# Yxxxb/LAVT-RS

Measured on NVIDIA B200. Metric: LAVT-RS fwd clips/s (8x384^2), higher is better.
Workload: dtype bf16

## Files before the change

### include/lavt_b200.h

```cpp
#ifndef LAVT_B200_H_
#define LAVT_B200_H_

#include <stdint.h>

#ifdef __cplusplus
extern "C" {
#endif

#define LAVT_ABI_VERSION 4

#define LAVT_ERR_SHAPE 1
#define LAVT_ERR_CUDA 2
#define LAVT_ERR_ARCH 3

enum { LAVT_ACT_NONE = 0, LAVT_ACT_GELU = 1, LAVT_ACT_RELU = 2, LAVT_ACT_TANH = 3, LAVT_ACT_SIGMOID = 4 };

typedef struct lavt_win_geom {
  int32_t B, D, H, W;
  int32_t wd, wh, ww;
  int32_t sd, sh, sw;
  int32_t nwd, nwh, nww;
  int32_t N;
  int32_t Wd, Wh, Ww;
} lavt_win_geom_t;

typedef struct lavt_epilogue {
  const float* cscale;
  const float* bias;
  int32_t act;
  int32_t ldm;
  const void* mul;
  const float* resid;
  float* out_f32;
  void* out_bf16;
  int32_t ldo;
  int32_t mul_act;
  const lavt_win_geom_t* win;
  const float* rscale;
  int32_t rscale_rows;
  int32_t pre_mode;
  void* out_pre;
} lavt_epilogue_t;

const char* lavt_last_error(void);
int lavt_abi_version(void);
int lavt_check_device(void);

int lavt_gemm_bf16(const void* A, int64_t lda, const void* Wt, int64_t ldw, int32_t M, int32_t N, int32_t K,
                   const lavt_epilogue_t* epi, void* stream);

int lavt_conv3x3_bf16(const void* x_nhwc, int64_t ldx, int32_t n_img, int32_t H, int32_t W, int32_t Cin,
                      const void* Wt, int32_t Cout, const lavt_epilogue_t* epi, void* stream);

int lavt_conv3d_bf16(const void* x_ndhwc, int64_t ldx, int32_t n_clip, int32_t D, int32_t H, int32_t W, int32_t Cin,
                     const void* Wt, int32_t Cout, const lavt_epilogue_t* epi, void* stream);


int lavt_layernorm_rows(const float* x, int64_t ldx, int64_t M, int32_t C, const float* gamma, const float* beta,
                        float eps, void* out_bf16, float* out_f32, void* stream);

int lavt_layernorm_window_gather(const float* x, int32_t C, const lavt_win_geom_t* geom, const float* gamma,
                                 const float* beta, float eps, void* out_bf16, void* stream);

int lavt_patch_merge_layernorm(const float* x, int32_t B, int32_t D, int32_t H, int32_t W, int32_t C,
                               const float* gamma, const float* beta, float eps, void* out_bf16, void* stream);

int lavt_patch_embed_im2col(const float* x, int64_t stride_b, int64_t stride_c, int64_t stride_t, int32_t B, int32_t T,
                            int32_t H, int32_t W, void* out_bf16, void* stream);

int lavt_window_attention(const void* qkv, const float* table_t, int32_t L, int32_t nH, const lavt_win_geom_t* geom,
                          void* out_bf16, void* stream);
int lavt_window_attention_lse(const void* qkv, const float* table_t, int32_t L, int32_t nH, const lavt_win_geom_t* geom, void* out_bf16,
                              float* lse, void* stream);
int lavt_window_attention_has_lse(const lavt_win_geom_t* geom, int32_t L, int32_t nH);
int lavt_set_attention_impl(int32_t impl);

int64_t lavt_instnorm_workspace_floats(int32_t B, int64_t n, int32_t C);
int lavt_instnorm_stats(const float* x, int32_t B, int64_t n, int32_t C, float eps, float* stats,
                        float* workspace, void* stream);
int lavt_pwam_kv(const float* l, const float* mask, const float* wk, const float* bk, const float* wv, const float* bv,
                 float* k, float* v, int32_t B, int32_t Nl, int32_t Lin, int32_t C, void* stream);
int lavt_lang_project(const float* l, const float* mask, const float* w0, const float* b0, const float* w2, const float* b2, float* stats,
// ... 157 lines not shown
```

### lavt_rs_b200/_cabi.py

```python
from __future__ import annotations

import ctypes as C
import os
from typing import Optional

import torch

_PKG = os.path.dirname(os.path.abspath(__file__))
LIB_PATH = os.environ.get("LAVT_LIB_PATH") or os.path.join(_PKG, "_lib", "liblavt_b200.so")

ACT_NONE, ACT_GELU, ACT_RELU, ACT_TANH, ACT_SIGMOID = 0, 1, 2, 3, 4


class WinGeom(C.Structure):
    _fields_ = [(n, C.c_int32) for n in
                ("B", "D", "H", "W", "wd", "wh", "ww", "sd", "sh", "sw",
                 "nwd", "nwh", "nww", "N", "Wd", "Wh", "Ww")]

    def rows(self) -> int:
        return self.B * self.nwd * self.nwh * self.nww * self.N

    def tokens(self) -> int:
        return self.B * self.D * self.H * self.W

# ... 14 lines not shown
class LavtError(RuntimeError):
    pass


_lib: Optional[C.CDLL] = None


def lib() -> C.CDLL:
    global _lib
    if _lib is not None:
        return _lib
    if not os.path.exists(LIB_PATH):
        raise LavtError(
            f"{LIB_PATH} not found: build it with `python -m lavt_rs_b200.build` "
            "(the B200 path has no CPU / PyTorch fallback)")
    l = C.CDLL(LIB_PATH)
    l.lavt_last_error.restype = C.c_char_p
    _declare(l)
    if l.lavt_abi_version() != ABI_VERSION:
        raise LavtError("liblavt_b200.so ABI version mismatch; rebuild")
    _lib = l
    return l


ABI_VERSION = 4

_i32, _i64, _f32, _vp = C.c_int32, C.c_int64, C.c_float, C.c_void_p
_EP = C.POINTER(Epilogue)
_WG = C.POINTER(WinGeom)

SIGNATURES = {
    "lavt_check_device": [],
    "lavt_gemm_bf16": [_vp, _i64, _vp, _i64, _i32, _i32, _i32, _EP, _vp],
    "lavt_gemm_bf16_smallm": [_vp, _i64, _vp, _i64, _i32, _i32, _i32, _EP, _vp, _i64, _vp],
    "lavt_conv3x3_bf16": [_vp, _i64, _i32, _i32, _i32, _i32, _vp, _i32, _EP, _vp],
    "lavt_conv3d_bf16": [_vp, _i64, _i32, _i32, _i32, _i32, _i32, _vp, _i32, _EP, _vp],
    "lavt_layernorm_rows": [_vp, _i64, _i64, _i32, _vp, _vp, _f32, _vp, _vp, _vp],
    "lavt_layernorm_window_gather": [_vp, _i32, _WG, _vp, _vp, _f32, _vp, _vp],
    "lavt_patch_merge_layernorm": [_vp, _i32, _i32, _i32, _i32, _i32, _vp, _vp, _f32, _vp, _vp],
    "lavt_patch_embed_im2col": [_vp, _i64, _i64, _i64, _i32, _i32, _i32, _i32, _vp, _vp],
    "lavt_window_attention": [_vp, _vp, _i32, _i32, _WG, _vp, _vp],
    "lavt_window_attention_lse": [_vp, _vp, _i32, _i32, _WG, _vp, _vp, _vp],
    "lavt_instnorm_stats": [_vp, _i32, _i64, _i32, _f32, _vp, _vp, _vp],
    "lavt_pwam_kv": [_vp, _vp, _vp, _vp, _vp, _vp, _vp, _vp, _i32, _i32, _i32, _i32, _vp],
    "lavt_lang_project": [_vp, _vp, _vp, _vp, _vp, _vp, _vp, _i32, _i32, _i32, _i32, _vp],
    "lavt_lang_project_bwd": [_vp, _vp, _vp, _vp, _vp, _vp, _vp, _vp, _vp, _vp, _vp, _vp, _i32, _i32, _i32, _i32, _vp],
    "lavt_pwam_attend": [_vp, _vp, _vp, _vp, _vp, _vp, _i32, _i64, _i32, _i32, _i32, _vp],
    "lavt_pwam_mul_norm": [_vp, _vp, _vp, _vp, _i32, _i64, _i32, _vp],
    "lavt_instnorm_sum2": [_vp, _vp, _vp, _vp, _vp, _i32, _i64, _i32, _vp],
    "lavt_bert_embed": [_vp, _vp, _vp, _vp, _vp, _i32, _i32, _i32, _i32, _vp],
    "lavt_bert_attention": [_vp, _vp, _vp, _i32, _i32, _i32, _i32, _vp],
    "lavt_rows_to_channels_first": [_vp, _vp, _i32, _i32, _i32, _vp],
    "lavt_split3_bf16": [_vp, _i64, _vp, _i64, _i32, _vp],
    "lavt_bert_attention_f32": [_vp, _vp, _vp, _i32, _i32, _i32, _i32, _vp],
    "lavt_upsample_concat": [_vp, _i32, _i32, _i32, _vp, _i32, _vp, _i32, _i32, _i32, _vp],
    "lavt_upconv_blend": [_vp, _i32, _i32, _i32, _vp, _vp, _vp, _vp, _i32, _i32, _i32, _vp],
    "lavt_conv1x1_logits": [_vp, _vp, _vp, _vp, _i64, _i32, _vp],
    "lavt_upsample_logits": [_vp, _vp, _i32, _i32, _i32, _i32, _i32, _vp],
    "lavt_nhwc_to_nchw": [_vp, _vp, _i32, _i32, _i32, _vp],
    "lavt_nchw_to_nhwc_bf16": [_vp, _vp, _i32, _i32, _i32, _vp],
    "lavt_gemm_bf16_splitk": [_vp, _i64, _vp, _i64, _i32, _i32, _i32, _i32, _vp, _i64, _vp, _i64, _i32, _vp],
    "lavt_gemm_bf16_wgrad": [_vp, _i64, _vp, _i64, _i64, _i32, _i32, _vp, _i64, _vp, _i64, _i32, _vp],
    "lavt_conv3x3_wgrad": [_vp, _vp, _i32, _i32, _i32, _i32, _i32, _vp, _i64, _vp, _i32, _vp],
    "lavt_conv3d_wgrad": [_vp, _vp, _i32, _i32, _i32, _i32, _i32, _i32, _vp, _i64, _vp, _i32, _vp],
    "lavt_transpose_bf16": [_vp, _i64, _vp, _i64, _i64, _i32, _vp],
    "lavt_colsum_accumulate": [_vp, _i32, _i64, _i64, _i32, _vp, _vp],
# ... 175 lines not shown
        torch.cuda.synchronize()
        out = {}
        for fam, fl, nb, s, e, _tag in self.records:
            d = out.setdefault(fam, {"launches": 0, "ms": 0.0, "flops": 0.0, "bytes": 0.0, "ideal_ms": 0.0})
            d["launches"] += 1
            d["ms"] += s.elapsed_time(e)
            d["flops"] += fl
            d["bytes"] += nb
            if peak_tflops > 0 and peak_gbs > 0:
                d["ideal_ms"] += max(fl / (peak_tflops * 1e12), nb / (peak_gbs * 1e9)) * 1e3
        return out


TIMER = KernelTimer()


def gemm_bf16(a: torch.Tensor, w: torch.Tensor, **epi) -> None:
    _req(a, torch.bfloat16, "a")
    _req(w, torch.bfloat16, "w")
    M, K = a.shape
    N, K2 = w.shape
    if K != K2:
        raise LavtError(f"gemm: K mismatch {K} vs {K2}")
    e = make_epilogue(**epi)
    t0 = TIMER.begin()
    check(lib().lavt_gemm_bf16(a.data_ptr(), a.stride(0), w.data_ptr(), w.stride(0), M, N, K,
                               C.byref(e), stream_ptr()), "lavt_gemm_bf16")
    if t0 is not None:
        nbytes = 2.0 * (M * K + N * K) + M * N * ((4.0 if e.out_f32 else 0.0) + (2.0 if e.out_bf16 else 0.0)
                                                   + (4.0 if e.resid else 0.0) + (2.0 if e.mul else 0.0))
        TIMER.end(t0, "gemm_bf16_tc_kernel", 2.0 * M * N * K, nbytes, f"M{M} N{N} K{K} act{e.act}")


def gemm_bf16_smallm(a: torch.Tensor, w: torch.Tensor, workspace: torch.Tensor, **epi) -> None:
    _req(a, torch.bfloat16, "a")
    _req(w, torch.bfloat16, "w")
    M, K = a.shape
    N, K2 = w.shape
    if K != K2:
        raise LavtError(f"gemm: K mismatch {K} vs {K2}")
    e = make_epilogue(**epi)
    check(lib().lavt_gemm_bf16_smallm(a.data_ptr(), a.stride(0), w.data_ptr(), w.stride(0), M, N, K, C.byref(e),
                                      _c(workspace, torch.float32, "workspace").data_ptr(), workspace.numel(), stream_ptr()),
          "lavt_gemm_bf16_smallm")


def conv3x3_bf16(x_nhwc: torch.Tensor, w_taps: torch.Tensor, **epi) -> None:
    _req(x_nhwc, torch.bfloat16, "x")
    _req(w_taps, torch.bfloat16, "w_taps")
    n_img, H, W, Cin = x_nhwc.shape
    if not x_nhwc.is_contiguous():
        raise LavtError("conv: x must be contiguous NHWC")
    Cout = w_taps.shape[0]
    e = make_epilogue(**epi)
    t0 = TIMER.begin()
    check(lib().lavt_conv3x3_bf16(x_nhwc.data_ptr(), Cin, n_img, H, W, Cin, w_taps.data_ptr(), Cout,
                                  C.byref(e), stream_ptr()), "lavt_conv3x3_bf16")
    npix = n_img * H * W
    TIMER.end(t0, "gemm_bf16_tc_kernel", 2.0 * npix * Cout * 9 * Cin, 2.0 * (npix * Cin + Cout * 9 * Cin + npix * Cout),
              f"conv {n_img}x{H}x{W} Cin{Cin} Cout{Cout}")


def conv3d_bf16(x_ndhwc: torch.Tensor, w_taps: torch.Tensor, **epi) -> None:
    _req(x_ndhwc, torch.bfloat16, "x")
    _req(w_taps, torch.bfloat16, "w_taps")
    n_clip, D, H, W, Cin = x_ndhwc.shape
# ... 778 lines not shown
```

### lavt_rs_b200/csrc/cabi.cu

```cuda
#include "../../include/lavt_b200.h"
#include "common.cuh"
#include "gemm_tc.cuh"
#include "kernels.cuh"

#include <cstring>

namespace lavt {
const char* last_error();
int gemm_dispatch(const void* A, long long lda, const void* Bw, long long ldb, const GemmParams& p,
                  cudaStream_t stream);

static_assert(sizeof(lavt_win_geom_t) == sizeof(WinGeom), "public/private window geometry mismatch");

static int fill_epilogue(GemmParams& p, const lavt_epilogue_t* e) {
  LAVT_REQUIRE(e != nullptr, "epilogue pointer is NULL");
  p.cscale = e->cscale;
  p.bias = e->bias;
  p.act = e->act;
  p.mul = static_cast<const __nv_bfloat16*>(e->mul);
  p.ldm = e->ldm;
  p.mul_act = e->mul_act;
  p.out_pre = static_cast<__nv_bfloat16*>(e->out_pre);
  p.pre_mode = e->pre_mode;
  LAVT_REQUIRE(e->pre_mode == 0 || (e->pre_mode == 1 && e->out_pre && e->act == LAVT_ACT_GELU),
               "epilogue: pre_mode 1 (out_pre = GELU'(pre)) needs out_pre and act = LAVT_ACT_GELU");
  LAVT_REQUIRE(e->mul_act == 0 || (e->mul_act == LAVT_ACT_GELU && e->mul), "epilogue: mul_act must be 0 or LAVT_ACT_GELU with a mul operand");
  p.resid = e->resid;
  p.out_f32 = e->out_f32;
  p.out_bf16 = static_cast<__nv_bfloat16*>(e->out_bf16);
  p.ldo = e->ldo;
  p.rscale = e->rscale;
  p.rs_rows = e->rscale_rows;
  LAVT_REQUIRE(!e->rscale || e->rscale_rows > 0, "epilogue: rscale needs rscale_rows > 0");
  LAVT_REQUIRE(e->act >= 0 && e->act <= 4, "bad activation id %d", e->act);
  if (e->win) {
    p.rowmap = ROWMAP_WINDOW;
    std::memcpy(&p.win, e->win, sizeof(WinGeom));
  } else {
    p.rowmap = ROWMAP_IDENTITY;
  }
  return LAVT_OK;
}
}
// ... 2 lines not shown

extern "C" {

const char* lavt_last_error(void) { return lavt::last_error(); }
int lavt_abi_version(void) { return LAVT_ABI_VERSION; }

int lavt_check_device(void) {
  int dev = 0;
  LAVT_CUDA(cudaGetDevice(&dev));
  cudaDeviceProp prop;
  LAVT_CUDA(cudaGetDeviceProperties(&prop, dev));
  if (prop.major != 10) {
    set_last_error("device %d is sm_%d%d; this library is built for sm_100a only", dev, prop.major, prop.minor);
    return LAVT_ERR_ARCH;
  }
  return LAVT_OK;
}

int lavt_gemm_bf16(const void* A, int64_t lda, const void* Wt, int64_t ldw, int32_t M, int32_t N, int32_t K,
                   const lavt_epilogue_t* epi, void* stream) {
  GemmParams p;
  std::memset(&p, 0, sizeof(p));
  p.M = M; p.N = N; p.K = K;
  int rc = fill_epilogue(p, epi);
  if (rc) return rc;
  if (p.rowmap == ROWMAP_WINDOW) {
    const WinGeom& g = p.win;
    long long rows = 1LL * g.B * g.nwd * g.nwh * g.nww * g.N;
    LAVT_REQUIRE(rows == M, "gemm: window geometry rows %lld != M %d", rows, M);
  }
  return gemm_dispatch(A, lda, Wt, ldw, p, static_cast<cudaStream_t>(stream));
}

static void conv_pick_tile(GemmParams& p, int H, int W) {
  int best_tw = 8; long long best_area = -1;
  for (int tw = 8; tw <= 128; tw *= 2) {
    int th = 128 / tw;
    long long area = 1LL * ((H + th - 1) / th) * th * ((W + tw - 1) / tw) * tw;
    if (best_area < 0 || area < best_area || (area == best_area && tw > best_tw)) { best_area = area; best_tw = tw; }
  }
  p.cTW = best_tw; p.cTH = 128 / best_tw;
  p.cTilesW = (W + p.cTW - 1) / p.cTW;
  p.cTilesH = (H + p.cTH - 1) / p.cTH;
}

int lavt_conv3x3_bf16(const void* x_nhwc, int64_t ldx, int32_t n_img, int32_t H, int32_t W, int32_t Cin,
                      const void* Wt, int32_t Cout, const lavt_epilogue_t* epi, void* stream) {
  GemmParams p;
  std::memset(&p, 0, sizeof(p));
  LAVT_REQUIRE(n_img > 0 && H > 0 && W > 0, "conv: empty input");
  p.M = n_img * H * W; p.N = Cout; p.K = 9 * Cin;
  int rc = fill_epilogue(p, epi);
  if (rc) return rc;
  LAVT_REQUIRE(p.rowmap == ROWMAP_IDENTITY, "conv: window row map not applicable");
  p.rowmap = ROWMAP_CONV;
  p.cH = H; p.cW = W; p.cCin = Cin; p.taps = 9;
  conv_pick_tile(p, H, W);
  return gemm_dispatch(x_nhwc, ldx, Wt, 9LL * Cin, p, static_cast<cudaStream_t>(stream));
}

int lavt_conv3d_bf16(const void* x_ndhwc, int64_t ldx, int32_t n_clip, int32_t D, int32_t H, int32_t W, int32_t Cin,
                     const void* Wt, int32_t Cout, const lavt_epilogue_t* epi, void* stream) {
  GemmParams p;
  std::memset(&p, 0, sizeof(p));
  LAVT_REQUIRE(n_clip > 0 && D > 0 && H > 0 && W > 0, "conv3d: empty input");
  LAVT_REQUIRE(1LL * n_clip * D * H * W < (1LL << 31), "conv3d: too many output positions");
// ... 489 lines not shown
```

### lavt_rs_b200/csrc/gemm_tc.cu

```cuda
#include "common.cuh"
#include "gemm_tc.cuh"

#include <cstdio>
#include <cstdlib>
#include <cstring>

namespace lavt {

constexpr int GEMM_BM = 128;
constexpr int GEMM_BK = 64;

template <int GEMM_BN, int GEMM_STAGES, int EPI_WGS, int CTA2 = 0>
struct GemmSmem {
  static constexpr int A_BYTES = GEMM_BM * GEMM_BK * 2;
  static constexpr int B_BYTES = (CTA2 ? GEMM_BN / 2 : GEMM_BN) * GEMM_BK * 2;
  static constexpr int STAGE_BYTES = A_BYTES + B_BYTES;
  static constexpr int RING_BYTES = GEMM_STAGES * STAGE_BYTES;
  static constexpr int BAR_OFF = RING_BYTES;
  static constexpr int VEC_OFF = BAR_OFF + 256;
  static constexpr int VEC_TILE_BYTES = EPI_WGS * 2 * GEMM_BN * 4;
  static constexpr int TOTAL = VEC_OFF + VEC_TILE_BYTES + 1024 ;
  static constexpr int THREADS = 128 + 128 * EPI_WGS;
  static constexpr int MIN_CTAS = (EPI_WGS == 1) ? 2 : 1;
  static constexpr int ACC = (MIN_CTAS == 2) ? 2 : 512 / GEMM_BN;
};

__device__ __forceinline__ float ex2_approx(float x) {
  float y;
  asm("ex2.approx.ftz.f32 %0, %1;" : "=f"(y) : "f"(x));
  return y;
}
__device__ __forceinline__ float rcp_approx(float x) {
  float y;
  asm("rcp.approx.ftz.f32 %0, %1;" : "=f"(y) : "f"(x));
  return y;
}
__device__ __forceinline__ uint64_t pk2(float lo, float hi) {
  uint64_t r;
  asm("mov.b64 %0, {%1, %2};" : "=l"(r) : "f"(lo), "f"(hi));
  return r;
}
__device__ __forceinline__ void upk2(uint64_t v, float& lo, float& hi) { asm("mov.b64 {%0, %1}, %2;" : "=f"(lo), "=f"(hi) : "l"(v)); }
__device__ __forceinline__ uint64_t fma2(uint64_t a, uint64_t b, uint64_t c) {
  uint64_t r;
  asm("fma.rn.f32x2 %0, %1, %2, %3;" : "=l"(r) : "l"(a), "l"(b), "l"(c));
  return r;
}
__device__ __forceinline__ uint64_t mul2(uint64_t a, uint64_t b) {
  uint64_t r;
  asm("mul.rn.f32x2 %0, %1, %2;" : "=l"(r) : "l"(a), "l"(b));
  return r;
}
__device__ __forceinline__ void gelu_erf2(float& x0, float& x1) {
  const uint64_t x = pk2(x0, x1);
  float z0, z1;
  upk2(mul2(x, pk2(0.70710678118654752f, 0.70710678118654752f)), z0, z1);
  z0 = fminf(fmaxf(z0, -3.0f), 3.0f);
  z1 = fminf(fmaxf(z1, -3.0f), 3.0f);
  const uint64_t z = pk2(z0, z1);
  const uint64_t t = mul2(z, z);
  constexpr float K = 1.0000220904f;
  uint64_t p = pk2(4.0742095563e-08f * K, 4.0742095563e-08f * K);
  p = fma2(p, t, pk2(-1.9448222676e-06f * K, -1.9448222676e-06f * K));
  p = fma2(p, t, pk2(4.1060515983e-05f * K, 4.1060515983e-05f * K));
  p = fma2(p, t, pk2(-5.1103678896e-04f * K, -5.1103678896e-04f * K));
  p = fma2(p, t, pk2(4.2354270142e-03f * K, 4.2354270142e-03f * K));
  p = fma2(p, t, pk2(-2.5102860078e-02f * K, -2.5102860078e-02f * K));
  p = fma2(p, t, pk2(1.1107933337e-01f * K, 1.1107933337e-01f * K));
  p = fma2(p, t, pk2(-3.7531487405e-01f * K, -3.7531487405e-01f * K));
  p = fma2(p, t, pk2(1.1282684285e+00f * K, 1.1282684285e+00f * K));
  const uint64_t e = mul2(z, p);
  const uint64_t hx = mul2(x, pk2(0.5f, 0.5f));
  upk2(fma2(hx, e, hx), x0, x1);
}
__device__ __forceinline__ void gelu_both2(float& x0, float& x1, float& d0, float& d1) {
  const uint64_t x = pk2(x0, x1);
  float z0, z1;
  upk2(mul2(x, pk2(0.70710678118654752f, 0.70710678118654752f)), z0, z1);
  const uint64_t zz = pk2(z0, z1);
  float q0, q1;
  upk2(mul2(zz, zz), q0, q1);
  const float e0 = ex2_approx(-1.4426950408889634f * q0), e1 = ex2_approx(-1.4426950408889634f * q1);
  z0 = fminf(fmaxf(z0, -3.0f), 3.0f);
  z1 = fminf(fmaxf(z1, -3.0f), 3.0f);
  const uint64_t z = pk2(z0, z1);
  const uint64_t t = mul2(z, z);
  constexpr float K = 1.0000220904f;
  uint64_t p = pk2(4.0742095563e-08f * K, 4.0742095563e-08f * K);
  p = fma2(p, t, pk2(-1.9448222676e-06f * K, -1.9448222676e-06f * K));
  p = fma2(p, t, pk2(4.1060515983e-05f * K, 4.1060515983e-05f * K));
  p = fma2(p, t, pk2(-5.1103678896e-04f * K, -5.1103678896e-04f * K));
  p = fma2(p, t, pk2(4.2354270142e-03f * K, 4.2354270142e-03f * K));
  p = fma2(p, t, pk2(-2.5102860078e-02f * K, -2.5102860078e-02f * K));
  p = fma2(p, t, pk2(1.1107933337e-01f * K, 1.1107933337e-01f * K));
  p = fma2(p, t, pk2(-3.7531487405e-01f * K, -3.7531487405e-01f * K));
  p = fma2(p, t, pk2(1.1282684285e+00f * K, 1.1282684285e+00f * K));
  const uint64_t Phi = fma2(mul2(z, p), pk2(0.5f, 0.5f), pk2(0.5f, 0.5f));
  const uint64_t xs = mul2(x, pk2(0.3989422804014327f, 0.3989422804014327f));
  upk2(fma2(xs, pk2(e0, e1), Phi), d0, d1);
  upk2(mul2(x, Phi), x0, x1);
}
__device__ __forceinline__ void gelu_grad2(float& x0, float& x1) {
  float d0, d1;
  gelu_both2(x0, x1, d0, d1);
  x0 = d0;
  x1 = d1;
}
__device__ __forceinline__ void ldg_v8(uint32_t* r, const void* p) {
  asm volatile("ld.global.v8.b32 {%0, %1, %2, %3, %4, %5, %6, %7}, [%8];"
               : "=r"(r[0]), "=r"(r[1]), "=r"(r[2]), "=r"(r[3]), "=r"(r[4]), "=r"(r[5]), "=r"(r[6]), "=r"(r[7])
               : "l"(p));
}
__device__ __forceinline__ void stg_v8(void* p, const uint32_t* r) {
  asm volatile("st.global.v8.b32 [%0], {%1, %2, %3, %4, %5, %6, %7, %8};" ::"l"(p), "r"(r[0]), "r"(r[1]), "r"(r[2]),
               "r"(r[3]), "r"(r[4]), "r"(r[5]), "r"(r[6]), "r"(r[7])
               : "memory");
}
__device__ __forceinline__ float tanh_fast(float x) {
  const float e = ex2_approx(x * 2.8853900817779268f);
  return fmaf(-2.0f, rcp_approx(e + 1.0f), 1.0f);
}

template <int GEMM_BN, int GEMM_STAGES, int EPI_WGS, int CTA2 = 0, int SIMPLE = 0>
__global__ void __launch_bounds__(GemmSmem<GEMM_BN, GEMM_STAGES, EPI_WGS, CTA2>::THREADS, GemmSmem<GEMM_BN, GEMM_STAGES, EPI_WGS, CTA2>::MIN_CTAS)
gemm_bf16_tc_kernel(const __grid_constant__ CUtensorMap tmA, const __grid_constant__ CUtensorMap tmB,
                    const GemmParams p, const int m_tiles, const int vec_all, long long* const trace_buf) {
  using L = GemmSmem<GEMM_BN, GEMM_STAGES, EPI_WGS, CTA2>;
  const int crank = CTA2 ? static_cast<int>(cluster_ctarank()) : 0;
  const int wid0 = CTA2 ? static_cast<int>(blockIdx.x >> 1) : static_cast<int>(blockIdx.x);
  const int wstep = CTA2 ? static_cast<int>(gridDim.x >> 1) : static_cast<int>(gridDim.x);
  extern __shared__ uint8_t smem_raw[];
  uint8_t* smem = smem_raw + ((1024u - (smem_u32(smem_raw) & 1023u)) & 1023u);
  uint64_t* full_bar = reinterpret_cast<uint64_t*>(smem + L::BAR_OFF);
  uint64_t* empty_bar = full_bar + GEMM_STAGES;
  constexpr int ACC = L::ACC;
  uint64_t* tmem_full_bar = empty_bar + GEMM_STAGES;
  uint64_t* tmem_empty_bar = tmem_full_bar + ACC;
  uint32_t* tmem_ptr_smem = reinterpret_cast<uint32_t*>(tmem_empty_bar + ACC);

  const int warp = threadIdx.x >> 5;
  const int lane = threadIdx.x & 31;
  long long* const trace = (blockIdx.x == 0) ? trace_buf : nullptr;
#define GEMM_TRACE(ev, lt) do { if (trace && (lt) < 32) trace[(ev) * 32 + (lt)] = clock64(); } while (0)
  const int n_tiles = (p.N + GEMM_BN - 1) / GEMM_BN;
  const int total_tiles = (CTA2 ? (m_tiles + 1) / 2 : m_tiles) * n_tiles;
  const int conv_cpb = (p.cCin + GEMM_BK - 1) / GEMM_BK;
  const int num_kb = (p.rowmap == ROWMAP_CONV) ? p.taps * conv_cpb
                     : (p.rowmap == ROWMAP_WGCONV) ? (p.K / GEMM_BK) : (p.K + GEMM_BK - 1) / GEMM_BK;
  const int nsplit = p.ksplit > 1 ? p.ksplit : 1;
  const int kbs = p.ksplit > 1 ? p.kbs : num_kb;
// ... 558 lines not shown
```

### lavt_rs_b200/csrc/gemm_tc.cuh

```cuda
#pragma once
#include "geom.cuh"
#include <cuda_bf16.h>

namespace lavt {

enum GemmAct { ACT_NONE = 0, ACT_GELU = 1, ACT_RELU = 2, ACT_TANH = 3, ACT_SIGMOID = 4 };
enum GemmRowMap { ROWMAP_IDENTITY = 0, ROWMAP_WINDOW = 1, ROWMAP_CONV = 2, ROWMAP_WGCONV = 3 };

struct GemmParams {
  int M, N, K;
  const float* cscale;
  const float* bias;
  int act;
  const __nv_bfloat16* mul;
  int ldm;
  int mul_act;
  __nv_bfloat16* out_pre;
  int pre_mode;
  const float* resid;
  float* out_f32;
  __nv_bfloat16* out_bf16;
  int ldo;
  const float* rscale;
  int rs_rows;
  int rowmap;
  WinGeom win;
  int cH, cW, cCin;
  int cTH, cTW;
  int cTilesH, cTilesW;
  int taps;
  int cD;
  int ksplit;
  int kbs;
  long long split_stride;
  int mnmajor;
  int b_koff;
};
int splitk_epilogue_dispatch(const float* partials, int splits, long long M, int N, const float* cscale, const float* bias, int act,
                             const float* resid, float* out_f32, __nv_bfloat16* out_bf16, long long ldo, cudaStream_t st);
int splitk_reduce_dispatch(const float* partials, int splits, long long count, int ncols, float* dst, long long ldd, int accumulate,
                           cudaStream_t st);

}
```

### lavt_rs_b200/engine.py

```python
from __future__ import annotations

from typing import Dict, Optional, Sequence, Tuple

import torch

from . import _cabi as K
from .geometry import window_geometry

LAUNCHES = 0
PRECISION = "bf16"


def set_precision(mode: str) -> str:
    global PRECISION
    if mode not in ("bf16", "fp32"):
        raise ValueError("precision must be 'bf16' or 'fp32'")
    prev, PRECISION = PRECISION, mode
    return prev


def _count(n: int = 1) -> None:
    global LAUNCHES
    LAUNCHES += n

# ... 29 lines not shown
    return _WORKSPACES[key]


class PreparedWeights:

    def __init__(self):
        self._cache: Dict[str, Tuple[tuple, object]] = {}

    def get(self, key: str, sources: Sequence[torch.Tensor], build):
        ver = tuple((t.data_ptr(), t._version, t.device) for t in sources)
        hit = self._cache.get(key)
        if hit is not None and hit[0] == ver:
            return hit[1]
        with torch.no_grad():
            val = build()
        self._cache[key] = (ver, val)
        return val

    def clear(self):
        self._cache.clear()


def _bf16(t: torch.Tensor) -> torch.Tensor:
    return t.detach().to(torch.bfloat16).contiguous()


def _f32(t: torch.Tensor) -> torch.Tensor:
    return t.detach().to(torch.float32).contiguous()


def require_cuda(t: torch.Tensor, what: str) -> None:
    if not t.is_cuda:
        raise K.LavtError(f"{what} must live on a CUDA device: the B200 path has no CPU fallback")


def swin_block(x: torch.Tensor, blk, B: int, D: int, H: int, W: int, window, shifted: bool, clamp: bool,
               ws: Workspace, xb_out: Optional[torch.Tensor] = None) -> None:
    n, C = x.shape
    dev = x.device
    geom = window_geometry(B, D, H, W, window, shifted, clamp)
    rows = geom.rows()
    nH = blk.num_heads
    pw = blk.prepared
    hd = C // nH
    if PRECISION == "fp32":
        return _swin_block_fp32(x, blk, geom, ws, xb_out)

    qkv_w = pw.get("qkv_w", [blk.attn.qkv.weight], lambda: _bf16(blk.attn.qkv.weight))
    def _qscale():
        s = torch.ones(3 * C, device=dev, dtype=torch.float32)
        s[:C] = hd ** -0.5 * 1.4426950408889634
        b = _f32(blk.attn.qkv.bias) * s if blk.attn.qkv.bias is not None else torch.zeros(3 * C, device=dev)
        return s, b
    qkv_s, qkv_b = pw.get("qkv_sb", [blk.attn.qkv.weight] + ([blk.attn.qkv.bias] if blk.attn.qkv.bias is not None else []), _qscale)
    proj_w = pw.get("proj_w", [blk.attn.proj.weight], lambda: _bf16(blk.attn.proj.weight))
    fc1_w = pw.get("fc1_w", [blk.mlp.fc1.weight], lambda: _bf16(blk.mlp.fc1.weight))
    fc2_w = pw.get("fc2_w", [blk.mlp.fc2.weight], lambda: _bf16(blk.mlp.fc2.weight))
    table_t = pw.get("table_t", [blk.attn.relative_position_bias_table],
                     lambda: _f32(blk.attn.relative_position_bias_table.t()))

    xw = ws.get("xw", (rows, C), torch.bfloat16, dev)
    K.layernorm_window_gather(x, geom, blk.norm1.weight, blk.norm1.bias, xw, eps=blk.norm1.eps)
    qkv = ws.get("qkv", (rows, 3 * C), torch.bfloat16, dev)
    K.gemm_bf16(xw, qkv_w, cscale=qkv_s, bias=qkv_b, out_bf16=qkv)
    att = ws.get("att", (rows, C), torch.bfloat16, dev)
    K.window_attention(qkv, table_t, geom, att)
    K.gemm_bf16(att, proj_w, bias=blk.attn.proj.bias.detach(), resid=x, out_f32=x, win=geom)
    h1 = ws.get("ln2", (n, C), torch.bfloat16, dev)
    K.layernorm_rows(x, blk.norm2.weight, blk.norm2.bias, out_bf16=h1, eps=blk.norm2.eps)
    hid = ws.get("hid", (n, fc1_w.shape[0]), torch.bfloat16, dev)
    K.gemm_bf16(h1, fc1_w, bias=blk.mlp.fc1.bias.detach(), act=K.ACT_GELU, out_bf16=hid)
    K.gemm_bf16(hid, fc2_w, bias=blk.mlp.fc2.bias.detach(), resid=x, out_f32=x, out_bf16=xb_out)
    _count(7)


def _swin_block_fp32(x: torch.Tensor, blk, geom, ws: Workspace, xb_out: Optional[torch.Tensor]) -> None:
    n, C = x.shape
    dev = x.device
    rows, nH = geom.rows(), blk.num_heads
    hd = C // nH
    s = torch.ones(3 * C, device=dev, dtype=torch.float32)
    s[:C] = hd ** -0.5 * 1.4426950408889634
    qb = _f32(blk.attn.qkv.bias) * s if blk.attn.qkv.bias is not None else torch.zeros(3 * C, device=dev)
    xw = ws.get("xw32", (rows, C), torch.float32, dev)
    K.layernorm_window_gather_f32(x, geom, blk.norm1.weight, blk.norm1.bias, xw, eps=blk.norm1.eps)
    qkv = ws.get("qkv32", (rows, 3 * C), torch.float32, dev)
    K.gemm_f32_ref(xw, _f32(blk.attn.qkv.weight), cscale=s, bias=qb, out_f32=qkv)
    att = ws.get("att32", (rows, C), torch.float32, dev)
    K.window_attention_f32_ref(qkv, _f32(blk.attn.relative_position_bias_table.t()), geom, att)
    K.gemm_f32_ref(att, _f32(blk.attn.proj.weight), bias=blk.attn.proj.bias.detach(), resid=x, out_f32=x, win=geom)
    h1 = ws.get("ln2_32", (n, C), torch.float32, dev)
    K.layernorm_rows(x, blk.norm2.weight, blk.norm2.bias, out_f32=h1, eps=blk.norm2.eps)
    hid = ws.get("hid32", (n, blk.mlp.fc1.weight.shape[0]), torch.float32, dev)
    K.gemm_f32_ref(h1, _f32(blk.mlp.fc1.weight), bias=blk.mlp.fc1.bias.detach(), act=K.ACT_GELU, out_f32=hid)
    K.gemm_f32_ref(hid, _f32(blk.mlp.fc2.weight), bias=blk.mlp.fc2.bias.detach(), resid=x, out_f32=x, out_bf16=xb_out)
    _count(7)


def _conv1x1_w(conv) -> torch.Tensor:
    return conv.weight[:, :, 0]


# ... 683 lines not shown
```

Baseline: 303.5.

## Fuse Swin MLP fc1-GELU-fc2 into one persistent tcgen05 kernel

Adds a persistent warp-specialized kernel that runs fc1, bias plus GELU, and fc2 with the residual add per 128-row tile. The hidden activation stays in TMEM and shared memory instead of being written to and reread from global memory. TMA weight loads are streamed through a ring buffer, and double-buffered TMEM accumulators let the GELU epilogue of one chunk overlap the MMAs of the next. It applies only to bf16 with C of 128 or 256; weights are re-streamed for every tile, and with a single CTA per SM the MMAs may stall waiting on the epilogue warps.

```diff
diff --git a/include/lavt_b200.h b/include/lavt_b200.h
--- a/include/lavt_b200.h
+++ b/include/lavt_b200.h
@@ -48,6 +48,9 @@
 
 int lavt_gemm_bf16(const void* A, int64_t lda, const void* Wt, int64_t ldw, int32_t M, int32_t N, int32_t K,
                    const lavt_epilogue_t* epi, void* stream);
+
+int lavt_swin_mlp_bf16(const void* h, int64_t ldh, const void* W1, const void* W2, const float* b1, const float* b2, float* x,
+                       void* xb_out, int64_t ldx, int64_t M, int32_t C, int32_t hidden, void* stream);
 
 int lavt_conv3x3_bf16(const void* x_nhwc, int64_t ldx, int32_t n_img, int32_t H, int32_t W, int32_t Cin,
                       const void* Wt, int32_t Cout, const lavt_epilogue_t* epi, void* stream);
diff --git a/lavt_rs_b200/_cabi.py b/lavt_rs_b200/_cabi.py
--- a/lavt_rs_b200/_cabi.py
+++ b/lavt_rs_b200/_cabi.py
@@ -70,6 +70,7 @@
 SIGNATURES = {
     "lavt_check_device": [],
     "lavt_gemm_bf16": [_vp, _i64, _vp, _i64, _i32, _i32, _i32, _EP, _vp],
+    "lavt_swin_mlp_bf16": [_vp, _i64, _vp, _vp, _vp, _vp, _vp, _vp, _i64, _i64, _i32, _i32, _vp],
     "lavt_gemm_bf16_smallm": [_vp, _i64, _vp, _i64, _i32, _i32, _i32, _EP, _vp, _i64, _vp],
     "lavt_conv3x3_bf16": [_vp, _i64, _i32, _i32, _i32, _i32, _vp, _i32, _EP, _vp],
     "lavt_conv3d_bf16": [_vp, _i64, _i32, _i32, _i32, _i32, _i32, _vp, _i32, _EP, _vp],
@@ -311,6 +312,31 @@
         TIMER.end(t0, "gemm_bf16_tc_kernel", 2.0 * M * N * K, nbytes, f"M{M} N{N} K{K} act{e.act}")
 
 
+def swin_mlp(h: torch.Tensor, w1: torch.Tensor, b1, w2: torch.Tensor, b2, x: torch.Tensor, xb_out=None) -> None:
+    if h.dtype == torch.float32:
+        raise LavtError("swin_mlp: fp32 operands (validation precision) run as two gemm_f32_ref calls; the fused MLP is bf16 only")
+    _req(h, torch.bfloat16, "h")
+    w1, w2 = _c(w1, torch.bfloat16, "w1"), _c(w2, torch.bfloat16, "w2")
+    _req(x, torch.float32, "x")
+    M, Cn = h.shape
+    hidden = w1.shape[0]
+    if tuple(w1.shape) != (hidden, Cn) or tuple(w2.shape) != (Cn, hidden) or tuple(x.shape) != (M, Cn):
+        raise LavtError(f"swin_mlp: shapes h {tuple(h.shape)} w1 {tuple(w1.shape)} w2 {tuple(w2.shape)} x {tuple(x.shape)} do not match")
+    if xb_out is not None:
+        _req(xb_out, torch.bfloat16, "xb_out")
+        if tuple(xb_out.shape) != (M, Cn) or xb_out.stride(0) != x.stride(0):
+            raise LavtError("swin_mlp: xb_out must be [M, C] with the row pitch of x")
+    b1p = _c(b1.detach(), torch.float32, "b1").data_ptr() if b1 is not None else None
+    b2p = _c(b2.detach(), torch.float32, "b2").data_ptr() if b2 is not None else None
+    t0 = TIMER.begin()
+    check(lib().lavt_swin_mlp_bf16(h.data_ptr(), h.stride(0), w1.data_ptr(), w2.data_ptr(), b1p, b2p, x.data_ptr(),
+                                   xb_out.data_ptr() if xb_out is not None else None, x.stride(0), M, Cn, hidden, stream_ptr()),
+          "lavt_swin_mlp_bf16")
+    if t0 is not None:
+        nbytes = 2.0 * M * Cn + 4.0 * Cn * hidden + 8.0 * M * Cn + (2.0 * M * Cn if xb_out is not None else 0.0)
+        TIMER.end(t0, "swin_mlp_tc_kernel", 4.0 * M * Cn * hidden, nbytes, f"M{M} C{Cn} hidden{hidden}")
+
+
 def gemm_bf16_smallm(a: torch.Tensor, w: torch.Tensor, workspace: torch.Tensor, **epi) -> None:
     _req(a, torch.bfloat16, "a")
     _req(w, torch.bfloat16, "w")
diff --git a/lavt_rs_b200/csrc/cabi.cu b/lavt_rs_b200/csrc/cabi.cu
--- a/lavt_rs_b200/csrc/cabi.cu
+++ b/lavt_rs_b200/csrc/cabi.cu
@@ -9,6 +9,8 @@
 const char* last_error();
 int gemm_dispatch(const void* A, long long lda, const void* Bw, long long ldb, const GemmParams& p,
                   cudaStream_t stream);
+int swin_mlp_dispatch(const void* A, long long lda, const void* W1, const void* W2, const float* b1, const float* b2, float* x,
+                      __nv_bfloat16* xb_out, long long ldo, long long M, int C, int hidden, cudaStream_t stream);
 
 static_assert(sizeof(lavt_win_geom_t) == sizeof(WinGeom), "public/private window geometry mismatch");
 
@@ -77,6 +79,12 @@
   return gemm_dispatch(A, lda, Wt, ldw, p, static_cast<cudaStream_t>(stream));
 }
 
+int lavt_swin_mlp_bf16(const void* h, int64_t ldh, const void* W1, const void* W2, const float* b1, const float* b2, float* x,
+                       void* xb_out, int64_t ldx, int64_t M, int32_t C, int32_t hidden, void* stream) {
+  return swin_mlp_dispatch(h, ldh, W1, W2, b1, b2, x, static_cast<__nv_bfloat16*>(xb_out), ldx, M, C, hidden,
+                           static_cast<cudaStream_t>(stream));
+}
+
 static void conv_pick_tile(GemmParams& p, int H, int W) {
   int best_tw = 8; long long best_area = -1;
   for (int tw = 8; tw <= 128; tw *= 2) {
diff --git a/lavt_rs_b200/csrc/gemm_tc.cu b/lavt_rs_b200/csrc/gemm_tc.cu
--- a/lavt_rs_b200/csrc/gemm_tc.cu
+++ b/lavt_rs_b200/csrc/gemm_tc.cu
@@ -34,44 +34,6 @@
   float y;
   asm("rcp.approx.ftz.f32 %0, %1;" : "=f"(y) : "f"(x));
   return y;
-}
-__device__ __forceinline__ uint64_t pk2(float lo, float hi) {
-  uint64_t r;
-  asm("mov.b64 %0, {%1, %2};" : "=l"(r) : "f"(lo), "f"(hi));
-  return r;
-}
-__device__ __forceinline__ void upk2(uint64_t v, float& lo, float& hi) { asm("mov.b64 {%0, %1}, %2;" : "=f"(lo), "=f"(hi) : "l"(v)); }
-__device__ __forceinline__ uint64_t fma2(uint64_t a, uint64_t b, uint64_t c) {
-  uint64_t r;
-  asm("fma.rn.f32x2 %0, %1, %2, %3;" : "=l"(r) : "l"(a), "l"(b), "l"(c));
-  return r;
-}
-__device__ __forceinline__ uint64_t mul2(uint64_t a, uint64_t b) {
-  uint64_t r;
-  asm("mul.rn.f32x2 %0, %1, %2;" : "=l"(r) : "l"(a), "l"(b));
-  return r;
-}
-__device__ __forceinline__ void gelu_erf2(float& x0, float& x1) {
-  const uint64_t x = pk2(x0, x1);
-  float z0, z1;
-  upk2(mul2(x, pk2(0.70710678118654752f, 0.70710678118654752f)), z0, z1);
-  z0 = fminf(fmaxf(z0, -3.0f), 3.0f);
-  z1 = fminf(fmaxf(z1, -3.0f), 3.0f);
-  const uint64_t z = pk2(z0, z1);
-  const uint64_t t = mul2(z, z);
-  constexpr float K = 1.0000220904f;
-  uint64_t p = pk2(4.0742095563e-08f * K, 4.0742095563e-08f * K);
-  p = fma2(p, t, pk2(-1.9448222676e-06f * K, -1.9448222676e-06f * K));
-  p = fma2(p, t, pk2(4.1060515983e-05f * K, 4.1060515983e-05f * K));
-  p = fma2(p, t, pk2(-5.1103678896e-04f * K, -5.1103678896e-04f * K));
-  p = fma2(p, t, pk2(4.2354270142e-03f * K, 4.2354270142e-03f * K));
-  p = fma2(p, t, pk2(-2.5102860078e-02f * K, -2.5102860078e-02f * K));
-  p = fma2(p, t, pk2(1.1107933337e-01f * K, 1.1107933337e-01f * K));
-  p = fma2(p, t, pk2(-3.7531487405e-01f * K, -3.7531487405e-01f * K));
-  p = fma2(p, t, pk2(1.1282684285e+00f * K, 1.1282684285e+00f * K));
-  const uint64_t e = mul2(z, p);
-  const uint64_t hx = mul2(x, pk2(0.5f, 0.5f));
-  upk2(fma2(hx, e, hx), x0, x1);
 }
 __device__ __forceinline__ void gelu_both2(float& x0, float& x1, float& d0, float& d1) {
   const uint64_t x = pk2(x0, x1);
@@ -106,16 +68,6 @@
   x0 = d0;
   x1 = d1;
 }
-__device__ __forceinline__ void ldg_v8(uint32_t* r, const void* p) {
-  asm volatile("ld.global.v8.b32 {%0, %1, %2, %3, %4, %5, %6, %7}, [%8];"
-               : "=r"(r[0]), "=r"(r[1]), "=r"(r[2]), "=r"(r[3]), "=r"(r[4]), "=r"(r[5]), "=r"(r[6]), "=r"(r[7])
-               : "l"(p));
-}
-__device__ __forceinline__ void stg_v8(void* p, const uint32_t* r) {
-  asm volatile("st.global.v8.b32 [%0], {%1, %2, %3, %4, %5, %6, %7, %8};" ::"l"(p), "r"(r[0]), "r"(r[1]), "r"(r[2]),
-               "r"(r[3]), "r"(r[4]), "r"(r[5]), "r"(r[6]), "r"(r[7])
-               : "memory");
-}
 __device__ __forceinline__ float tanh_fast(float x) {
   const float e = ex2_approx(x * 2.8853900817779268f);
   return fmaf(-2.0f, rcp_approx(e + 1.0f), 1.0f);
diff --git a/lavt_rs_b200/csrc/gemm_tc.cuh b/lavt_rs_b200/csrc/gemm_tc.cuh
--- a/lavt_rs_b200/csrc/gemm_tc.cuh
+++ b/lavt_rs_b200/csrc/gemm_tc.cuh
@@ -36,6 +36,57 @@
   int mnmajor;
   int b_koff;
 };
+#ifdef __CUDACC__
+__device__ __forceinline__ uint64_t pk2(float lo, float hi) {
+  uint64_t r;
+  asm("mov.b64 %0, {%1, %2};" : "=l"(r) : "f"(lo), "f"(hi));
+  return r;
+}
+__device__ __forceinline__ void upk2(uint64_t v, float& lo, float& hi) { asm("mov.b64 {%0, %1}, %2;" : "=f"(lo), "=f"(hi) : "l"(v)); }
+__device__ __forceinline__ uint64_t fma2(uint64_t a, uint64_t b, uint64_t c) {
+  uint64_t r;
+  asm("fma.rn.f32x2 %0, %1, %2, %3;" : "=l"(r) : "l"(a), "l"(b), "l"(c));
+  return r;
+}
+__device__ __forceinline__ uint64_t mul2(uint64_t a, uint64_t b) {
+  uint64_t r;
+  asm("mul.rn.f32x2 %0, %1, %2;" : "=l"(r) : "l"(a), "l"(b));
+  return r;
+}
+__device__ __forceinline__ void gelu_erf2(float& x0, float& x1) {
+  const uint64_t x = pk2(x0, x1);
+  float z0, z1;
+  upk2(mul2(x, pk2(0.70710678118654752f, 0.70710678118654752f)), z0, z1);
+  z0 = fminf(fmaxf(z0, -3.0f), 3.0f);
+  z1 = fminf(fmaxf(z1, -3.0f), 3.0f);
+  const uint64_t z = pk2(z0, z1);
+  const uint64_t t = mul2(z, z);
+  constexpr float K = 1.0000220904f;
+  uint64_t p = pk2(4.0742095563e-08f * K, 4.0742095563e-08f * K);
+  p = fma2(p, t, pk2(-1.9448222676e-06f * K, -1.9448222676e-06f * K));
+  p = fma2(p, t, pk2(4.1060515983e-05f * K, 4.1060515983e-05f * K));
+  p = fma2(p, t, pk2(-5.1103678896e-04f * K, -5.1103678896e-04f * K));
+  p = fma2(p, t, pk2(4.2354270142e-03f * K, 4.2354270142e-03f * K));
+  p = fma2(p, t, pk2(-2.5102860078e-02f * K, -2.5102860078e-02f * K));
+  p = fma2(p, t, pk2(1.1107933337e-01f * K, 1.1107933337e-01f * K));
+  p = fma2(p, t, pk2(-3.7531487405e-01f * K, -3.7531487405e-01f * K));
+  p = fma2(p, t, pk2(1.1282684285e+00f * K, 1.1282684285e+00f * K));
+  const uint64_t e = mul2(z, p);
+  const uint64_t hx = mul2(x, pk2(0.5f, 0.5f));
+  upk2(fma2(hx, e, hx), x0, x1);
+}
+__device__ __forceinline__ void ldg_v8(uint32_t* r, const void* p) {
+  asm volatile("ld.global.v8.b32 {%0, %1, %2, %3, %4, %5, %6, %7}, [%8];"
+               : "=r"(r[0]), "=r"(r[1]), "=r"(r[2]), "=r"(r[3]), "=r"(r[4]), "=r"(r[5]), "=r"(r[6]), "=r"(r[7])
+               : "l"(p));
+}
+__device__ __forceinline__ void stg_v8(void* p, const uint32_t* r) {
+  asm volatile("st.global.v8.b32 [%0], {%1, %2, %3, %4, %5, %6, %7, %8};" ::"l"(p), "r"(r[0]), "r"(r[1]), "r"(r[2]),
+               "r"(r[3]), "r"(r[4]), "r"(r[5]), "r"(r[6]), "r"(r[7])
+               : "memory");
+}
+#endif
+
 int splitk_epilogue_dispatch(const float* partials, int splits, long long M, int N, const float* cscale, const float* bias, int act,
                              const float* resid, float* out_f32, __nv_bfloat16* out_bf16, long long ldo, cudaStream_t st);
 int splitk_reduce_dispatch(const float* partials, int splits, long long count, int ncols, float* dst, long long ldd, int accumulate,
diff --git a/lavt_rs_b200/csrc/mlp_tc.cu b/lavt_rs_b200/csrc/mlp_tc.cu
--- /dev/null
+++ b/lavt_rs_b200/csrc/mlp_tc.cu
@@ -0,0 +1,365 @@
+#include "common.cuh"
+#include "gemm_tc.cuh"
+
+#include <cstdlib>
+
+namespace lavt {
+
+template <int C>
+struct MlpCfg {
+  static constexpr int HID = 4 * C;
+  static constexpr int HC = 128;
+  static constexpr int NCH = HID / HC;
+  static constexpr int STAGES = (C == 128) ? 6 : 5;
+  static constexpr int SLOT = 16384;
+  static constexpr int NP = C * HC * 2 / SLOT;
+  static constexpr int APP = 128 / HC;
+  static constexpr int GA = HC / 64;
+  static constexpr int A_BYTES = 128 * C * 2;
+  static constexpr int G_BYTES = 128 * HC * 2;
+  static constexpr int A_OFF = 0;
+  static constexpr int G_OFF = A_OFF + A_BYTES;
+  static constexpr int RING_OFF = G_OFF + 2 * G_BYTES;
+  static constexpr int B1_OFF = RING_OFF + STAGES * SLOT;
+  static constexpr int B2_OFF = B1_OFF + HID * 4;
+  static constexpr int BAR_OFF = B2_OFF + C * 4;
+  static constexpr int TOTAL = BAR_OFF + 256 + 1024 ;
+  static constexpr int THREADS = 640;
+  static constexpr int EPI_WARPS = 16;
+  static constexpr int HCOLS = HC / 4;
+  static constexpr int OCOLS = C / 4;
+  static constexpr uint32_t TMEM_COLS = 512;
+  static_assert(TOTAL <= 227 * 1024, "shared memory");
+  static_assert(C + 2 * HC <= 512, "TMEM");
+};
+
+template <int C>
+__global__ void __launch_bounds__(640, 1)
+swin_mlp_tc_kernel(const __grid_constant__ CUtensorMap tmA, const __grid_constant__ CUtensorMap tmW1,
+                   const __grid_constant__ CUtensorMap tmW2, const float* __restrict__ b1, const float* __restrict__ b2, float* x,
+                   __nv_bfloat16* xb_out, const long long ldo, const int M, const int m_tiles, const int AHEAD) {
+  using L = MlpCfg<C>;
+  constexpr int HC = L::HC, NCH = L::NCH, S = L::STAGES;
+  extern __shared__ uint8_t smem_raw[];
+  uint8_t* smem = smem_raw + ((1024u - (smem_u32(smem_raw) & 1023u)) & 1023u);
+  uint64_t* full_bar = reinterpret_cast<uint64_t*>(smem + L::BAR_OFF);
+  uint64_t* empty_bar = full_bar + S;
+  uint64_t* a_full = empty_bar + S;
+  uint64_t* a_empty = a_full + 1;
+  uint64_t* h_full = a_empty + 1;
+  uint64_t* h_empty = h_full + 2;
+  uint64_t* g_full = h_empty + 2;
+  uint64_t* g_empty = g_full + 2;
+  uint64_t* o_full = g_empty + 2;
+  uint64_t* o_empty = o_full + 1;
+  uint32_t* tmem_ptr_smem = reinterpret_cast<uint32_t*>(o_empty + 1);
+  float* s_b1 = reinterpret_cast<float*>(smem + L::B1_OFF);
+  float* s_b2 = reinterpret_cast<float*>(smem + L::B2_OFF);
+
+  const int warp = threadIdx.x >> 5;
+  const int lane = threadIdx.x & 31;
+
+  if (warp == 0 && lane == 0) {
+    tma_prefetch_desc(&tmA);
+    tma_prefetch_desc(&tmW1);
+    tma_prefetch_desc(&tmW2);
+  }
+  if (warp == 1 && lane == 0) {
+    for (int s = 0; s < S; ++s) {
+      mbar_init(&full_bar[s], 1);
+      mbar_init(&empty_bar[s], 1);
+    }
+    mbar_init(a_full, 1);
+    mbar_init(a_empty, 1);
+    for (int b = 0; b < 2; ++b) {
+      mbar_init(&h_full[b], 1);
+      mbar_init(&h_empty[b], L::EPI_WARPS);
+      mbar_init(&g_full[b], L::EPI_WARPS);
+      mbar_init(&g_empty[b], 1);
+    }
+    mbar_init(o_full, 1);
+    mbar_init(o_empty, L::EPI_WARPS);
+    fence_mbar_init();
+  }
+  if (warp == 2) tmem_alloc(tmem_ptr_smem, L::TMEM_COLS);
+  pdl_wait();
+  pdl_launch_dependents();
+  for (int i = threadIdx.x; i < L::HID; i += blockDim.x) s_b1[i] = b1 ? __ldg(b1 + i) : 0.0f;
+  for (int i = threadIdx.x; i < C; i += blockDim.x) s_b2[i] = b2 ? __ldg(b2 + i) : 0.0f;
+  tc_fence_before();
+  __syncthreads();
+  tc_fence_after();
+  const uint32_t tmem_base = *tmem_ptr_smem;
+  const uint32_t tmem_o = tmem_base;
+  const uint32_t tmem_h = tmem_base + C;
+  const int n_chunks = (m_tiles - static_cast<int>(blockIdx.x) + static_cast<int>(gridDim.x) - 1) / static_cast<int>(gridDim.x) * NCH;
+
+  if (warp == 0) {
+    if (lane == 0) {
+      int it = 0;
+      auto slot = [&](int& i) -> uint8_t* {
+        const int s = i % S;
+        mbar_wait(&empty_bar[s], ((i / S) & 1) ^ 1);
+        mbar_expect_tx(&full_bar[s], L::SLOT);
+        return smem + L::RING_OFF + s * L::SLOT;
+      };
+      auto load_w1 = [&](int j) {
+        for (int p = 0; p < L::NP; ++p, ++it) {
+          uint8_t* dst = slot(it);
+          for (int a = 0; a < L::APP; ++a)
+            tma_load_2d(dst + a * HC * 128, &tmW1, &full_bar[it % S], (p * L::APP + a) * 64, j * HC);
+        }
+      };
+      auto load_w2 = [&](int j) {
+        for (int p = 0; p < L::NP; ++p, ++it) {
+          uint8_t* dst = slot(it);
+          tma_load_2d(dst, &tmW2, &full_bar[it % S], j * HC + (p % L::GA) * 64, (p / L::GA) * 128);
+        }
+      };
+      auto w1 = [&](int g) {
+        const int lt = g / NCH, j = g - lt * NCH;
+        if (j == 0) {
+          mbar_wait(a_empty, (lt & 1) ^ 1);
+          mbar_expect_tx(a_full, L::A_BYTES);
+          const int tile = blockIdx.x + lt * gridDim.x;
+          for (int a = 0; a < C / 64; ++a) tma_load_2d(smem + L::A_OFF + a * 16384, &tmA, a_full, a * 64, tile * 128);
+        }
+        load_w1(j);
+      };
+      for (int g = 0; g < AHEAD && g < n_chunks; ++g) w1(g);
+      for (int g = 0; g < n_chunks; ++g) {
+        if (g + AHEAD < n_chunks) w1(g + AHEAD);
+        load_w2(g % NCH);
+      }
+    }
+  } else if (warp == 1) {
+    if (lane == 0) {
+      constexpr uint32_t idesc_h = make_idesc_bf16_f32(128, HC);
+      constexpr uint32_t idesc_o = make_idesc_bf16_f32(128, 128);
+      int it = 0;
+      const uint32_t sa = smem_u32(smem + L::A_OFF);
+      const uint32_t sg = smem_u32(smem + L::G_OFF);
+      auto fc1 = [&](int j, int c) {
+        const int b = c & 1;
+        mbar_wait(&h_empty[b], ((c >> 1) & 1) ^ 1);
+        tc_fence_after();
+        for (int p = 0; p < L::NP; ++p, ++it) {
+          const int s = it % S;
+          mbar_wait(&full_bar[s], (it / S) & 1);
+          tc_fence_after();
+          const uint32_t ss = smem_u32(smem + L::RING_OFF + s * L::SLOT);
+#pragma unroll
+          for (int a = 0; a < L::APP; ++a) {
+            const uint64_t da = make_kmajor_sw128_desc(sa + (p * L::APP + a) * 16384);
+            const uint64_t db = make_kmajor_sw128_desc(ss + a * HC * 128);
+#pragma unroll
+            for (int k = 0; k < 4; ++k) umma_bf16_ss(tmem_h + b * HC, da + 2 * k, db + 2 * k, idesc_h, (p | a | k) != 0);
+          }
+          umma_commit(&empty_bar[s]);
+        }
+        umma_commit(&h_full[b]);
+        if (j == NCH - 1) umma_commit(a_empty);
+      };
+      auto fc2 = [&](int j, int c) {
+        const int b = c & 1;
+        mbar_wait(&g_full[b], (c >> 1) & 1);
+        tc_fence_after();
+        for (int p = 0; p < L::NP; ++p, ++it) {
+          const int s = it % S;
+          mbar_wait(&full_bar[s], (it / S) & 1);
+          tc_fence_after();
+          const int ga = p % L::GA, ob = p / L::GA;
+          const uint64_t da = make_kmajor_sw128_desc(sg + b * L::G_BYTES + ga * 16384);
+          const uint64_t db = make_kmajor_sw128_desc(smem_u32(smem + L::RING_OFF + s * L::SLOT));
+#pragma unroll
+          for (int k = 0; k < 4; ++k) umma_bf16_ss(tmem_o + ob * 128, da + 2 * k, db + 2 * k, idesc_o, (j | ga | k) != 0);
+          umma_commit(&empty_bar[s]);
+        }
+        umma_commit(&g_empty[b]);
+      };
+      auto f1 = [&](int g) {
+        const int lt = g / NCH, j = g - lt * NCH;
+        if (j == 0) {
+          mbar_wait(a_full, lt & 1);
+          tc_fence_after();
+        }
+        fc1(j, g);
+      };
+      for (int g = 0; g < AHEAD && g < n_chunks; ++g) f1(g);
+      for (int g = 0; g < n_chunks; ++g) {
+        if (g + AHEAD < n_chunks) f1(g + AHEAD);
+        const int lt = g / NCH, j = g - lt * NCH;
+        if (j == 0) {
+          mbar_wait(o_empty, (lt & 1) ^ 1);
+          tc_fence_after();
+        }
+        fc2(j, g);
+        if (j == NCH - 1) umma_commit(o_full);
+      }
+    }
+  } else if (warp >= 4) {
+    const int wg = (warp - 4) >> 2;
+    const int ew = warp & 3;
+    const int r = ew * 32 + lane;
+    const uint32_t lane_off = static_cast<uint32_t>(ew * 32) << 16;
+    uint8_t* const g_base = smem + L::G_OFF;
+    int gc = 0, lt = 0;
+    for (int tile = blockIdx.x; tile < m_tiles; tile += gridDim.x, ++lt) {
+      const long long m = static_cast<long long>(tile) * 128 + r;
+      const bool live = m < M;
+      float* const x_row = live ? x + m * ldo : nullptr;
+      if (live) {
+#pragma unroll
+        for (int q = 0; q < L::OCOLS; q += 32) asm volatile("prefetch.global.L2 [%0];" ::"l"(x_row + wg * L::OCOLS + q));
+      }
+#pragma unroll 1
+      for (int j = 0; j < NCH; ++j, ++gc) {
+        const int b = gc & 1;
+        const uint32_t ph = (gc >> 1) & 1;
+        uint32_t v[L::HCOLS];
+        mbar_wait(&h_full[b], ph);
+        tc_fence_after();
+        const uint32_t taddr = tmem_h + b * HC + wg * L::HCOLS + lane_off;
+        if constexpr (L::HCOLS == 32) tmem_ld_32x32b_x32(taddr, v);
+        else tmem_ld_32x32b_x16(taddr, v);
+        tmem_ld_wait();
+        tc_fence_before();
+        __syncwarp();
+        if (lane == 0) mbar_arrive(&h_empty[b]);
+        const float4* bi4 = reinterpret_cast<const float4*>(s_b1 + j * HC + wg * L::HCOLS);
+        uint32_t u[L::HCOLS / 2];
+#pragma unroll
+        for (int q = 0; q < L::HCOLS / 4; ++q) {
+          const float4 bi = bi4[q];
+          float f0 = __uint_as_float(v[4 * q]) + bi.x, f1 = __uint_as_float(v[4 * q + 1]) + bi.y;
+          float f2 = __uint_as_float(v[4 * q + 2]) + bi.z, f3 = __uint_as_float(v[4 * q + 3]) + bi.w;
+          gelu_erf2(f0, f1);
+          gelu_erf2(f2, f3);
+          u[2 * q] = pack_bf16x2(f0, f1);
+          u[2 * q + 1] = pack_bf16x2(f2, f3);
+        }
+        mbar_wait(&g_empty[b], ph ^ 1);
+        const int col0 = wg * L::HCOLS;
+        uint8_t* const grow = g_base + b * L::G_BYTES + (col0 / 64) * 16384 + r * 128;
+#pragma unroll
+        for (int q = 0; q < L::HCOLS / 8; ++q) {
+          const int c16 = ((col0 % 64) / 8 + q) ^ (r & 7);
+          *reinterpret_cast<uint4*>(grow + c16 * 16) = make_uint4(u[4 * q], u[4 * q + 1], u[4 * q + 2], u[4 * q + 3]);
+        }
+        fence_proxy_async_smem();
+        __syncwarp();
+        if (lane == 0) mbar_arrive(&g_full[b]);
+      }
+#pragma unroll 1
+      for (int c = 0; c < L::OCOLS / 16; ++c) {
+        const int col = wg * L::OCOLS + c * 16;
+        uint32_t rr[16];
+        if (live) {
+          ldg_v8(&rr[0], x_row + col);
+          ldg_v8(&rr[8], x_row + col + 8);
+        }
+        if (c == 0) {
+          mbar_wait(o_full, lt & 1);
+          tc_fence_after();
+        }
+        uint32_t v[16];
+        tmem_ld_32x32b_x16(tmem_o + col + lane_off, v);
+        tmem_ld_wait();
+        if (c == L::OCOLS / 16 - 1) {
+          tc_fence_before();
+          __syncwarp();
+          if (lane == 0) mbar_arrive(o_empty);
+        }
+        if (!live) continue;
+        float f[16];
+        const float4* bi4 = reinterpret_cast<const float4*>(s_b2 + col);
+#pragma unroll
+        for (int q = 0; q < 4; ++q) {
+          const float4 bi = bi4[q];
+          f[4 * q] = (__uint_as_float(v[4 * q]) + bi.x) + __uint_as_float(rr[4 * q]);
+          f[4 * q + 1] = (__uint_as_float(v[4 * q + 1]) + bi.y) + __uint_as_float(rr[4 * q + 1]);
+          f[4 * q + 2] = (__uint_as_float(v[4 * q + 2]) + bi.z) + __uint_as_float(rr[4 * q + 2]);
+          f[4 * q + 3] = (__uint_as_float(v[4 * q + 3]) + bi.w) + __uint_as_float(rr[4 * q + 3]);
+        }
+#pragma unroll
+        for (int q = 0; q < 2; ++q) {
+          uint32_t w[8];
+#pragma unroll
+          for (int e = 0; e < 8; ++e) w[e] = __float_as_uint(f[q * 8 + e]);
+          stg_v8(x_row + col + q * 8, w);
+        }
+        if (xb_out) {
+          uint32_t w[8];
+#pragma unroll
+          for (int e = 0; e < 8; ++e) w[e] = pack_bf16x2(f[2 * e], f[2 * e + 1]);
+          stg_v8(xb_out + m * ldo + col, w);
+        }
+      }
+    }
+  }
+
+  tc_fence_before();
+  __syncthreads();
+  if (warp == 2) {
+    tc_fence_after();
+    tmem_dealloc(tmem_base, L::TMEM_COLS);
+  }
+}
+
+template <int C>
+static int launch_mlp(const void* A, long long lda, const void* W1, const void* W2, const float* b1, const float* b2, float* x,
+                      __nv_bfloat16* xb_out, long long ldo, int M, cudaStream_t stream) {
+  using L = MlpCfg<C>;
+  CUtensorMap tmA, tmW1, tmW2;
+  {
+    uint64_t dims[2] = {(uint64_t)C, (uint64_t)M};
+    uint64_t strides[1] = {(uint64_t)lda * 2};
+    uint32_t box[2] = {64, 128};
+    int rc = make_tmap_bf16(&tmA, A, 2, dims, strides, box, CU_TENSOR_MAP_SWIZZLE_128B);
+    if (rc) return rc;
+  }
+  {
+    uint64_t dims[2] = {(uint64_t)C, (uint64_t)L::HID};
+    uint64_t strides[1] = {(uint64_t)C * 2};
+    uint32_t box[2] = {64, (uint32_t)L::HC};
+    int rc = make_tmap_bf16(&tmW1, W1, 2, dims, strides, box, CU_TENSOR_MAP_SWIZZLE_128B);
+    if (rc) return rc;
+  }
+  {
+    uint64_t dims[2] = {(uint64_t)L::HID, (uint64_t)C};
+    uint64_t strides[1] = {(uint64_t)L::HID * 2};
+    uint32_t box[2] = {64, 128};
+    int rc = make_tmap_bf16(&tmW2, W2, 2, dims, strides, box, CU_TENSOR_MAP_SWIZZLE_128B);
+    if (rc) return rc;
+  }
+  auto kfn = swin_mlp_tc_kernel<C>;
+  static bool configured = false;
+  if (!configured) {
+    LAVT_CUDA(cudaFuncSetAttribute(kfn, cudaFuncAttributeMaxDynamicSharedMemorySize, L::TOTAL));
+    configured = true;
+  }
+  int dev = 0, sms = 0;
+  LAVT_CUDA(cudaGetDevice(&dev));
+  LAVT_CUDA(cudaDeviceGetAttribute(&sms, cudaDevAttrMultiProcessorCount, dev));
+  const int m_tiles = (M + 127) / 128;
+  const int grid = m_tiles < sms ? m_tiles : sms;
+  LAVT_CUDA(launch_pdl(kfn, dim3(grid), dim3(L::THREADS), L::TOTAL, stream, 1, tmA, tmW1, tmW2, b1, b2, x, xb_out, ldo, M, m_tiles, getenv("LAVT_MLP_AHEAD1") ? 1 : 2));
+  LAVT_LAUNCH_CHECK("swin_mlp_tc_kernel");
+  return LAVT_OK;
+}
+
+int swin_mlp_dispatch(const void* A, long long lda, const void* W1, const void* W2, const float* b1, const float* b2, float* x,
+                      __nv_bfloat16* xb_out, long long ldo, long long M, int C, int hidden, cudaStream_t stream) {
+  LAVT_REQUIRE(C == 128 || C == 256, "swin_mlp: C=%d not supported (the fused MLP takes C = 128 or 256; use the two fc GEMMs)", C);
+  LAVT_REQUIRE(hidden == 4 * C, "swin_mlp: hidden=%d must be 4 * C = %d", hidden, 4 * C);
+  LAVT_REQUIRE(M > 0 && M < (1LL << 31) - 128, "swin_mlp: M=%lld out of range", M);
+  LAVT_REQUIRE(A && W1 && W2 && x, "swin_mlp: NULL operand");
+  LAVT_REQUIRE(lda >= C && lda % 8 == 0, "swin_mlp: lda=%lld must be >= C and a multiple of 8", lda);
+  LAVT_REQUIRE(ldo >= C && ldo % 16 == 0, "swin_mlp: ldo=%lld must be >= C and a multiple of 16", ldo);
+  LAVT_REQUIRE((reinterpret_cast<uintptr_t>(x) | reinterpret_cast<uintptr_t>(xb_out)) % 32 == 0,
+               "swin_mlp: x / xb_out must be 32-byte aligned");
+  if (C == 128) return launch_mlp<128>(A, lda, W1, W2, b1, b2, x, xb_out, ldo, static_cast<int>(M), stream);
+  return launch_mlp<256>(A, lda, W1, W2, b1, b2, x, xb_out, ldo, static_cast<int>(M), stream);
+}
+
+}
diff --git a/lavt_rs_b200/engine.py b/lavt_rs_b200/engine.py
--- a/lavt_rs_b200/engine.py
+++ b/lavt_rs_b200/engine.py
@@ -85,6 +85,10 @@
 def require_cuda(t: torch.Tensor, what: str) -> None:
     if not t.is_cuda:
         raise K.LavtError(f"{what} must live on a CUDA device: the B200 path has no CPU fallback")
+
+
+def mlp_fused(C: int, hidden: int) -> bool:
+    return PRECISION == "bf16" and C in (128, 256) and hidden == 4 * C
 
 
 def swin_block(x: torch.Tensor, blk, B: int, D: int, H: int, W: int, window, shifted: bool, clamp: bool,
@@ -121,6 +125,10 @@
     K.gemm_bf16(att, proj_w, bias=blk.attn.proj.bias.detach(), resid=x, out_f32=x, win=geom)
     h1 = ws.get("ln2", (n, C), torch.bfloat16, dev)
     K.layernorm_rows(x, blk.norm2.weight, blk.norm2.bias, out_bf16=h1, eps=blk.norm2.eps)
+    if mlp_fused(C, fc1_w.shape[0]):
+        K.swin_mlp(h1, fc1_w, blk.mlp.fc1.bias, fc2_w, blk.mlp.fc2.bias, x, xb_out)
+        _count(6)
+        return
     hid = ws.get("hid", (n, fc1_w.shape[0]), torch.bfloat16, dev)
     K.gemm_bf16(h1, fc1_w, bias=blk.mlp.fc1.bias.detach(), act=K.ACT_GELU, out_bf16=hid)
     K.gemm_bf16(hid, fc2_w, bias=blk.mlp.fc2.bias.detach(), resid=x, out_f32=x, out_bf16=xb_out)
```

Measured after the change: 307.0 (median of 6 runs). 1.2% higher.
